# willi-menapace/PlayableEnvironments

Measured on AMD Instinct MI355X. Metric: Mrays/s, higher is better.
Workload: dtype f32; 1 GPU; tennis renderer, 256x256 frame per GPU (rank r renders the frame of seed 1234 + r), 4 objects, 64+128 hierarchical samples/ray (coarse+fine networks), eval - BASELINE.json configs[1]; rays_per_gpu=65536, frames_per_gpu=1, parallelism=frame shard x1

## Files before the change

### playableenvironments_amd/csrc/geometry.hip

```cpp
#include "pr_common.h"

namespace pr {

__global__ void k_camera_rays(int frames, int rays, int per_frame, float half_h, float half_w, const float* __restrict__ c2w,
                              const float* __restrict__ focals, const int32_t* __restrict__ rows,
                              const int32_t* __restrict__ cols, float* __restrict__ origins,
                              float* __restrict__ dirs, float* __restrict__ normals) {
    const long g = (long)blockIdx.x * blockDim.x + threadIdx.x;
    const long total = (long)frames * rays;
    if (g >= total) return;
    const int n = (int)(g / rays);
    const int r = (int)(g - (long)n * rays);
    const float* m = c2w + (size_t)n * 12;
    const float f = focals[n];
    const long pix = per_frame ? g : (long)r;
    const float dx = __fdiv_rn(__fsub_rn((float)cols[pix], half_w), f);
    const float dy = -__fdiv_rn(__fsub_rn((float)rows[pix], half_h), f);
    const float dz = -1.0f;
#pragma unroll
    for (int i = 0; i < 3; ++i) {
        const float v = __fadd_rn(__fadd_rn(__fmul_rn(dx, m[i * 4 + 0]), __fmul_rn(dy, m[i * 4 + 1])),
                                  __fmul_rn(dz, m[i * 4 + 2]));
        dirs[g * 3 + i] = v;
    }
// ... 185 lines not shown
__global__ __launch_bounds__(256) void k_scan_blocks_group(ScanGroup g) {
    scan_blocks_body(g.sums[blockIdx.x], g.offsets[blockIdx.x], g.total[blockIdx.x], g.n);
}

int launch_scan(const int32_t* sums, int32_t* offsets, int32_t* total, int n, hipStream_t s) {
    hipLaunchKernelGGL(k_scan_blocks, dim3(1), dim3(256), 0, s, sums, offsets, total, n);
    PR_LAUNCH_CHECK();
    return PR_OK;
}

__device__ __forceinline__ void fill_body(const FillParams& p) {
    __shared__ int lds[4];
    if (p.skip && *p.skip) return;
    const int lane = threadIdx.x & 63;
    const long g = (long)blockIdx.x * 256 + threadIdx.x;
    const long total = (long)p.frames * p.rays;
    const int P = p.positions;
    ObjRay ray = {};
    bool valid = false;
    int frame = 0;
    if (g < total) {
        const int n = frame = (int)(g / p.rays);
        const float* m = p.w2o + ((size_t)n * p.objects + p.object_index) * 12;
        ray = object_ray(m, p.ray_origins + (size_t)n * 3, p.ray_directions + (size_t)g * 3);
        valid = p.in_scene[(size_t)n * p.objects + p.object_index] != 0;
    }
    const long wave_first = g - lane;
    const RayLanes L(P, lane);
    auto walk = [&](auto&& per_ray) {
        for (int r0 = 0; r0 < 64 && wave_first + r0 < total; r0 += L.per_pass) {
            const int r = r0 + L.sub;
            per_ray(r0, r, wave_first + r < total, broadcast_ray(ray, valid, frame, r), (size_t)(wave_first + r) * P);
        }
    };
    auto inside_at = [&](bool live, const WaveRay& w, size_t base, int i, float* x, float* y, float* z) {
        if (!live || i >= P) return false;
        const float t = p.t[base + i];
        *x = __fadd_rn(w.o[0], __fmul_rn(w.d[0], t));
        *y = __fadd_rn(w.o[1], __fmul_rn(w.d[1], t));
        *z = __fadd_rn(w.o[2], __fmul_rn(w.d[2], t));
        return sample_kept(*x, *y, *z, p.lo, p.hi, p.occ, w.frame);
    };
    int count = 0;
    walk([&](int r0, int r, bool live, const WaveRay& w, size_t base) {
        int ray_count = 0;
        for (int i0 = 0; i0 < P; i0 += L.P2) {
            float x, y, z;
            ray_count += __popcll(L.mine(__ballot(inside_at(live, w, base, i0 + L.idx, &x, &y, &z))));
        }
        L.collect(ray_count, r0, lane, &count);
    });
    int block_total;
    const int first_slot = p.block_offsets[blockIdx.x] + block_exclusive_scan_256(count, lds, &block_total);
    walk([&](int r0, int r, bool live, const WaveRay& w, size_t base) {
        int slot = __shfl(first_slot, r, 64);
        for (int i0 = 0; i0 < P; i0 += L.P2) {
            const int i = i0 + L.idx;
            float x = 0.f, y = 0.f, z = 0.f;
            const bool inside = inside_at(live, w, base, i, &x, &y, &z);
            const unsigned long long mask = L.mine(__ballot(inside));
            if (inside) {
                const int mine = slot + __popcll(mask & ((1ull << L.idx) - 1ull));
                p.rec_pos[(size_t)mine * 3 + 0] = x;
                p.rec_pos[(size_t)mine * 3 + 1] = y;
                p.rec_pos[(size_t)mine * 3 + 2] = z;
                p.rec_flat[mine] = (int32_t)(base + i);
                p.slot[base + i] = mine;
            } else if (live && i < P) {
                p.slot[base + i] = -1;
            }
            slot += __popcll(mask);
        }
    });
}

__global__ __launch_bounds__(256) void k_fill(FillParams p) { fill_body(p); }
struct FillGroup { FillParams p[PR_MAX_OBJECTS]; };
__global__ __launch_bounds__(256) void k_fill_group(FillGroup g) { fill_body(g.p[blockIdx.y]); }

int launch_placement_group(const PlaceParams* pp, const FillParams* fp, int32_t* const* totals, int count, hipStream_t s) {
    if (count <= 0) return PR_OK;
    PR_REQUIRE(count <= PR_MAX_OBJECTS, "placement group: %d objects", count);
    static thread_local PlaceGroup pg;
    static thread_local FillGroup fg;
    ScanGroup sg;
    const long total = (long)pp[0].frames * pp[0].rays;
    const int blocks = (int)((total + 255) / 256);
    for (int k = 0; k < count; ++k) {
        pg.p[k] = pp[k];
        fg.p[k] = fp[k];
        sg.sums[k] = pp[k].block_sums;
        sg.offsets[k] = const_cast<int32_t*>(fp[k].block_offsets);
        sg.total[k] = totals[k];
    }
    sg.n = blocks;
    hipLaunchKernelGGL(k_place_coarse_group, dim3(blocks, count), dim3(256), 0, s, pg);
    PR_LAUNCH_CHECK();
    hipLaunchKernelGGL(k_scan_blocks_group, dim3(count), dim3(256), 0, s, sg);
    PR_LAUNCH_CHECK();
    hipLaunchKernelGGL(k_fill_group, dim3(blocks, count), dim3(256), 0, s, fg);
    PR_LAUNCH_CHECK();
    return PR_OK;
}

int launch_fill(const FillParams& p, hipStream_t s) {
    const long total = (long)p.frames * p.rays;
    const int blocks = (int)((total + 255) / 256);
    hipLaunchKernelGGL(k_fill, dim3(blocks), dim3(256), 0, s, p);
    PR_LAUNCH_CHECK();
    return PR_OK;
}

__device__ __forceinline__ void bitonic_sort_f32(float* key, int n , int lane) {
    for (int k = 2; k <= n; k <<= 1) {
        for (int j = k >> 1; j > 0; j >>= 1) {
            for (int i = lane; i < n; i += 64) {
                const int x = i ^ j;
                if (x > i) {
                    const float a = key[i], b = key[x];
                    const bool up = ((i & k) == 0);
                    if ((a > b) == up) {
                        key[i] = b;
                        key[x] = a;
                    }
                }
            }
            __syncthreads();
        }
    }
}

__global__ __launch_bounds__(64) void k_resample(ResampleParams p, int sort_size) {
    extern __shared__ float sm[];
    if (p.skip && *p.skip) return;
    const int Pc = p.pc, Pf = p.pf;
    float* tc = sm;
    float* al = tc + Pc;
    float* mids = al + Pc;
    float* cdf = mids + Pc;
    float* key = cdf + Pc;
    const int lane = threadIdx.x;
    const long g = blockIdx.x;
    const int n = (int)(g / p.rays);
    const float* m = p.w2o + ((size_t)n * p.objects + p.object_index) * 12;
    const ObjRay ray = object_ray(m, p.ray_origins + (size_t)n * 3, p.ray_directions + (size_t)g * 3);
    const bool valid = p.in_scene[(size_t)n * p.objects + p.object_index] != 0;
    const float norm = sqrtf(__fadd_rn(__fadd_rn(__fmul_rn(ray.d[0], ray.d[0]), __fmul_rn(ray.d[1], ray.d[1])),
                                       __fmul_rn(ray.d[2], ray.d[2])));
    const size_t cbase = (size_t)g * Pc;
    for (int i = lane; i < Pc; i += 64) tc[i] = p.t_coarse[cbase + i];
    __syncthreads();
    for (int i = lane; i < Pc; i += 64) {
        float raw = valid ? p.sigma_coarse[cbase + i] : p.empty_alpha;
        if (noise_present(p.alpha_noise)) raw = __fadd_rn(raw, noise_normal(p.alpha_noise, g, Pc, i));
        const float dt = (i < Pc - 1) ? __fsub_rn(tc[i + 1], tc[i]) : 1e10f;
        const float dist = __fmul_rn(dt, norm);
        const float relu = raw > 0.f ? raw : 0.f;
        al[i] = __fsub_rn(1.0f, expf(__fmul_rn(-relu, dist)));
        if (i < Pc - 1) mids[i] = __fdiv_rn(__fadd_rn(tc[i + 1], tc[i]), 2.0f);
    }
    __syncthreads();
    if (lane == 0) {
        float trans = 1.0f;
        for (int i = 0; i < Pc; ++i) {
            const float a = al[i];
            al[i] = __fmul_rn(a, trans);
            trans = __fmul_rn(trans, __fadd_rn(__fsub_rn(1.0f, a), 1e-10f));
        }
        const int nb = Pc - 2;
        float sum = 0.f;
        for (int j = 0; j < nb; ++j) sum = __fadd_rn(sum, __fadd_rn(al[j + 1], 1e-5f));
        float c = 0.f;
        cdf[0] = 0.f;
        for (int j = 0; j < nb; ++j) {
            c = __fadd_rn(c, __fdiv_rn(__fadd_rn(al[j + 1], 1e-5f), sum));
            cdf[j + 1] = c;
        }
    }
    __syncthreads();
    const int ncdf = Pc - 1;
    for (int i = lane; i < sort_size; i += 64) key[i] = (i < Pc) ? tc[i] : __builtin_inff();
    for (int f = lane; f < Pf; f += 64) {
        const float u = noise_present(p.u_random) ? noise_uniform(p.u_random, g, Pf, f) : p.u_fixed[f];
        int lo_i = 0, hi_i = ncdf;
        while (lo_i < hi_i) {
            const int mid = (lo_i + hi_i) >> 1;
            if (cdf[mid] > u) hi_i = mid; else lo_i = mid + 1;
        }
        const int below = lo_i - 1 < 0 ? 0 : lo_i - 1;
        const int above = lo_i > ncdf - 1 ? ncdf - 1 : lo_i;
        float den = __fsub_rn(cdf[above], cdf[below]);
        if (den < 1e-5f) den = 1.0f;
        const float frac = __fdiv_rn(__fsub_rn(u, cdf[below]), den);
        key[Pc + f] = __fadd_rn(mids[below], __fmul_rn(frac, __fsub_rn(mids[above], mids[below])));
    }
    __syncthreads();
    const int Pm = Pc + Pf;
    float* merged = key + sort_size;
    bool sorted = true;
    for (int i = lane; i + 1 < Pc; i += 64) sorted = sorted && (key[i] <= key[i + 1]);
    for (int f = lane; f + 1 < Pf; f += 64) sorted = sorted && (key[Pc + f] <= key[Pc + f + 1]);
    if (__ballot(sorted) == ~0ull) {
        for (int i = lane; i < Pc; i += 64) {
            const float t = key[i];
            int lo = 0, hi = Pf;
            while (lo < hi) {
                const int mid = (lo + hi) >> 1;
                if (key[Pc + mid] < t) lo = mid + 1; else hi = mid;
            }
            merged[i + lo] = t;
        }
        for (int f = lane; f < Pf; f += 64) {
            const float t = key[Pc + f];
            int lo = 0, hi = Pc;
            while (lo < hi) {
                const int mid = (lo + hi) >> 1;
                if (key[mid] <= t) lo = mid + 1; else hi = mid;
            }
            merged[f + lo] = t;
        }
        __syncthreads();
    } else {
        bitonic_sort_f32(key, sort_size, lane);
        merged = key;
    }
    const size_t fbase = (size_t)g * Pm;
    int count = 0;
    for (int i = lane; i < Pm; i += 64) {
        const float t = merged[i];
        p.t_fine[fbase + i] = t;
        p.sigma_fine[fbase + i] = p.empty_alpha;
        if (p.dispmag_fine) p.dispmag_fine[fbase + i] = 0.f;
        const float x = __fadd_rn(ray.o[0], __fmul_rn(ray.d[0], t));
        const float y = __fadd_rn(ray.o[1], __fmul_rn(ray.d[1], t));
        const float z = __fadd_rn(ray.o[2], __fmul_rn(ray.d[2], t));
        if (sample_kept(x, y, z, p.lo, p.hi, p.occ, n)) ++count;
    }
#pragma unroll
    for (int d = 32; d > 0; d >>= 1) count += __shfl_down(count, d, 64);
    if (lane == 0 && count) atomicAdd(&p.block_sums[g >> 8], count);
}

__global__ __launch_bounds__(256) void k_expected_positions(int frames, int rays, int objects, int object_index, int P,
                                                            const float* ray_origins, const float* ray_directions,
                                                            const float* w2o, const float* t, const float* weights,
                                                            const float* delta, float* expected) {
    const long g = (long)blockIdx.x * 256 + threadIdx.x;
    if (g >= (long)frames * rays) return;
    const int n = (int)(g / rays);
    const ObjRay ray = object_ray(w2o + ((size_t)n * objects + object_index) * 12, ray_origins + (size_t)n * 3,
                                  ray_directions + (size_t)g * 3);
    const size_t base = (size_t)g * P;
    float acc[3] = {0.f, 0.f, 0.f}, wsum = 0.f;
    for (int i = 0; i < P; ++i) {
        const float ti = t[base + i], w = weights[base + i];
        for (int a = 0; a < 3; ++a) {
            float x = __fadd_rn(ray.o[a], __fmul_rn(ray.d[a], ti));
            if (delta) x = __fadd_rn(x, delta[(base + i) * 3 + a]);
            acc[a] = __fadd_rn(acc[a], __fmul_rn(x, w));
        }
        wsum = __fadd_rn(wsum, w);
    }
    for (int a = 0; a < 3; ++a) expected[(size_t)g * 3 + a] = __fdiv_rn(acc[a], __fadd_rn(wsum, 1e-8f));
}

static int next_pow2(int v) {
    int r = 1;
    while (r < v) r <<= 1;
    return r;
}

int launch_resample(const ResampleParams& p, hipStream_t s) {
    PR_REQUIRE(p.pc >= 3, "hierarchical sampling needs at least 3 coarse positions (got %d)", p.pc);
    const long total = (long)p.frames * p.rays;
    const int nblocks256 = (int)((total + 255) / 256);
    PR_TRY(launch_zero_fill(p.block_sums, sizeof(int32_t) * nblocks256, s));
    int sort_size = next_pow2(p.pc + p.pf);
    if (sort_size < 64) sort_size = 64;
    const size_t lds = sizeof(float) * (4 * (size_t)p.pc + 2 * (size_t)sort_size);
    PR_REQUIRE(lds <= 64 * 1024, "resample: too many positions per ray (%d + %d)", p.pc, p.pf);
    hipLaunchKernelGGL(k_resample, dim3((unsigned)total), dim3(64), lds, s, p, sort_size);
    PR_LAUNCH_CHECK();
    return PR_OK;
}

}

extern "C" int pr_expected_positions(int32_t frames, int32_t rays, int32_t objects, int32_t object_index, int32_t positions,
                                     const float* ray_origins, const float* ray_directions, const float* w2o, const float* t,
                                     const float* weights, const float* delta, float* expected, void* stream) {
    PR_REQUIRE(frames > 0 && rays > 0 && positions > 0 && objects > 0 && object_index >= 0 && object_index < objects,
               "pr_expected_positions: bad sizes");
    PR_REQUIRE(ray_origins && ray_directions && w2o && t && weights && expected, "pr_expected_positions: NULL pointer");
    const long total = (long)frames * rays;
    hipLaunchKernelGGL(pr::k_expected_positions, dim3((unsigned)((total + 255) / 256)), dim3(256), 0, (hipStream_t)stream, frames,
                       rays, objects, object_index, positions, ray_origins, ray_directions, w2o, t, weights, delta, expected);
    PR_LAUNCH_CHECK();
    return PR_OK;
}

namespace pr {
struct PatchPixelsParams {
    int frames, objects, height, width, patch, nstrides;
    int strides[4];
    const float* boxes;
    const float* weights;
    const float* u;
    int32_t* rows; int32_t* cols;
    int rays;
};

__global__ __launch_bounds__(256) void k_patch_pixels(PatchPixelsParams p) {
    __shared__ int start[2];
    const int n = blockIdx.x;
    const int H = p.height, W = p.width, K = p.objects;
    const int s0 = p.strides[0], sm = p.strides[p.nstrides - 1];
    if (threadIdx.x < 64) {
        const int lane = threadIdx.x;
        float left[PR_MAX_OBJECTS], right[PR_MAX_OBJECTS], top[PR_MAX_OBJECTS], bottom[PR_MAX_OBJECTS], per[PR_MAX_OBJECTS];
        for (int k = 0; k < K; ++k) {
            const float* b = p.boxes + (size_t)n * 4 * K + k;
            left[k] = fminf(fmaxf(floorf(b[0] * W), 0.f), (float)W);
            top[k] = fminf(fmaxf(floorf(b[K] * H), 0.f), (float)H);
            right[k] = fminf(fmaxf(ceilf(b[2 * K] * W), 0.f), (float)W);
            bottom[k] = fminf(fmaxf(ceilf(b[3 * K] * H), 0.f), (float)H);
            per[k] = p.weights[k] / ((right[k] - left[k]) * (bottom[k] - top[k]));
        }
        auto prefix = [&](long i) -> double {
            const int r = (int)(i / W), c = (int)(i - (long)r * W);
            double acc = 0.0;
            for (int k = 0; k < K; ++k) {
                const double w = right[k] - left[k];
                const double full = fmin((double)r, (double)bottom[k]) - top[k];
                double count = full > 0.0 ? full * w : 0.0;
                if (r >= top[k] && r < bottom[k]) {
                    const double part = fmin((double)(c + 1), (double)right[k]) - left[k];
                    if (part > 0.0) count += part;
                }
                if (count > 0.0) acc += (double)per[k] * count;
            }
            return acc;
        };
        const long total_px = (long)H * W;
        const double total = prefix(total_px - 1);
        long idx = total_px - 1;
        if (total > 0.0 && total < 1e300) {
            const double target = (double)p.u[n] * total;
            long lo = 0, hi = total_px - 1;
            while (lo < hi) {
                const long step = (hi - lo + 64) / 64;
                long cand = lo + (long)(lane + 1) * step - 1;
                if (cand > hi) cand = hi;
                const unsigned long long reached = __ballot(prefix(cand) >= target);
                const int first = reached ? __ffsll((long long)reached) - 1 : 63;
                long part_hi = lo + (long)(first + 1) * step - 1;
                if (part_hi > hi) part_hi = hi;
                lo = lo + (long)first * step;
                hi = part_hi;
            }
            idx = lo;
        }
        const int half = ((p.patch * s0) / sm) / 2;
        int row = (int)(idx / W), col = (int)(idx - (long)row * W);
        row = min(max(row, half * sm), H - sm * (half - 1) - 1);
// ... 407 lines not shown
```

### playableenvironments_amd/csrc/pr_common.h

```cpp
#pragma once

#include <hip/hip_runtime.h>
#include <stdint.h>
#include <stdio.h>
#include <string.h>

#include "playrender.h"

namespace pr {

void set_error(const char* fmt, ...);

#define PR_CHECK_HIP(expr)                                                              \
    do {                                                                                \
        hipError_t _e = (expr);                                                         \
        if (_e != hipSuccess) {                                                         \
            pr::set_error("%s failed: %s (%s:%d)", #expr, hipGetErrorString(_e), __FILE__, __LINE__); \
            return PR_ERR_HIP;                                                          \
        }                                                                               \
    } while (0)

#define PR_REQUIRE(cond, ...)                                                           \
    do {                                                                                \
        if (!(cond)) {                                                                  \
// ... 191 lines not shown
    const float* ptr;
    unsigned int key0, key1;
    int generate;
    int rays, ray_offset, total_rays;
    const unsigned long long* seed_dev;
    unsigned long long salt;
};

__host__ __device__ static inline unsigned long long noise_mix(unsigned long long x) {
    x += 0x9E3779B97F4A7C15ull;
    x = (x ^ (x >> 30)) * 0xBF58476D1CE4E5B9ull;
    x = (x ^ (x >> 27)) * 0x94D049BB133111EBull;
    return x ^ (x >> 31);
}

static inline NoiseRef make_noise(const float* ptr, const pr_call_t& c, int kind, int type, int object) {
    NoiseRef n;
    memset(&n, 0, sizeof(n));
    n.ptr = ptr;
    n.rays = c.rays;
    n.ray_offset = c.noise_ray_offset;
    n.total_rays = c.noise_total_rays > 0 ? c.noise_total_rays : c.rays;
    if (!ptr && (c.flags & PR_FLAG_DEVICE_NOISE)) {
        n.salt = noise_mix((unsigned long long)(kind * 16 + type * 8 + object) + 1);
        const unsigned long long k = noise_mix(c.noise_seed ^ n.salt);
        n.key0 = (unsigned int)k;
        n.key1 = (unsigned int)(k >> 32);
        n.seed_dev = reinterpret_cast<const unsigned long long*>(c.noise_seed_device);
        n.generate = 1;
    }
    return n;
}

static inline NoiseRef perturb_noise(const float* ptr, const pr_call_t& c, int kind, int type, int object) {
    NoiseRef n = make_noise(ptr, c, kind, type, object);
    if (!(c.flags & PR_FLAG_PERTURB)) n.generate = 0;
    return n;
}

struct OccGrid {
    const uint32_t* bits;
    int n[3];
    int words;
    float scale[3];
};
int make_occ_grid(const pr_occupancy_grid_t* g, const pr_object_model_t& m, int object, const char* level, OccGrid* out);

struct PlaceParams {
    int frames, rays, positions, objects, object_index;
    const float* ray_origins;
    const float* ray_directions;
    const float* w2o;
    const uint8_t* in_scene;
    float lo[3], hi[3];
    float z_near_min, z_far_max, empty_alpha;
    const float* linspace;
    NoiseRef jitter;
    float* t;
    float* sigma;
    float* dispmag;
    int32_t* block_sums;
    OccGrid occ;
    const int32_t* skip;
};
int launch_place_coarse(const PlaceParams& p, hipStream_t s);

struct FillParams {
    int frames, rays, positions, objects, object_index;
    const float* ray_origins;
    const float* ray_directions;
    const float* w2o;
    const uint8_t* in_scene;
    float lo[3], hi[3];
    const float* t;
    const int32_t* block_offsets;
    float* rec_pos;
    int32_t* rec_flat;
    int32_t* slot;
    OccGrid occ;
    const int32_t* skip;
};
int launch_fill(const FillParams& p, hipStream_t s);
int launch_placement_group(const PlaceParams* pp, const FillParams* fp, int32_t* const* totals, int count, hipStream_t s);

int launch_scan(const int32_t* sums, int32_t* offsets, int32_t* total, int n, hipStream_t s);

struct ResampleParams {
    int frames, rays, objects, object_index;
    int pc, pf;
    const float* ray_origins;
    const float* ray_directions;
    const float* w2o;
    const uint8_t* in_scene;
    float lo[3], hi[3];
    float empty_alpha;
    const float* t_coarse;
    const float* sigma_coarse;
    NoiseRef alpha_noise;
    const float* u_fixed;
    NoiseRef u_random;
    float* t_fine;
    float* sigma_fine;
    float* dispmag_fine;
    int32_t* block_sums;
    OccGrid occ;
    const int32_t* skip;
};
int launch_resample(const ResampleParams& p, hipStream_t s);

struct FoldParams {
    int frames, objects, object_index;
    const float* style;
    int S;
    pr_linear_t affine1; const float* bn1_mean; const float* bn1_var;
    pr_linear_t affine4; const float* bn4_mean; const float* bn4_var;
    float eps;
    int W, Wpad, W2, W2pad;
    float* table;
    int row_floats;
};
int launch_adain_fold(const FoldParams& p, hipStream_t s);
int launch_adain_fold_group(const FoldParams* jobs, int count, hipStream_t s);

int launch_mlp(const MlpParams& p, int max_rows, bool naive, const pr_object_model_t* raw, hipStream_t s);
int launch_mlp_group(const MlpParams* host_jobs, const int* max_rows, int count, hipStream_t s);
int launch_mlp_split(const MlpParams& p, int max_rows, int terms, hipStream_t s);
int launch_mlp_split_group(const MlpParams* host_jobs, const int* max_rows, int count, int terms, hipStream_t s);
int launch_mlp_sigma(const MlpParams& p, int max_rows, hipStream_t s);
int launch_mlp_split_sigma(const MlpParams& p, int max_rows, int terms, hipStream_t s);

struct BnFinalizeParams {
    const double* stats;
    const int32_t* count;
    int width, width_pad;
    float momentum;
    float* running_mean;
    float* running_var;
    long long* num_batches_tracked;
    float* batch_mean;
    float* batch_var;
    int frozen;
};
int launch_bn_finalize(const BnFinalizeParams& p, hipStream_t s);

struct BnFoldJob {
    const double* stats; const int32_t* count; int width, width_pad; float momentum;
    float* running_mean; float* running_var; long long* num_batches_tracked;
    float* batch_mean; float* batch_var; int frozen;
    const float* style; int style_stride, S, frames;
    pr_linear_t affine; float eps;
    float* table; int row_floats, g_off, b_off;
    int32_t* normalised_out;
};
struct BnFoldJobs { BnFoldJob job[PR_MAX_OBJECTS]; };
int launch_bn_fold_group(const BnFoldJobs& jobs, int count, hipStream_t s);

struct DivChainJob {
    const int32_t* total; const int32_t* rec_flat; const int32_t* row_flags; const float* rec_pos;
    NoiseRef noise; int positions;
    const float* bin; int bin_pad, benc, b_octaves;
    const unsigned char* bbits; size_t bbits_stride;
    int BW, BWpad, b_count, b_skip;
    Seg seg0[PR_MAX_LAYERS]; Seg seg1;
    const float* w_out;
    const float* braw;
    float lo[3], hi[3];
    int canonical;
    float* div;
    int32_t* tile_counter;
};
bool div_chain_supported(int BWpad, int bin_pad);
int launch_div_chain_group(const DivChainJob* jobs, const long* max_rows, int count, hipStream_t s);

struct CompositeObject {
    const float* t;
    const float* sigma;
    const int32_t* slot;
    const float* divergence;
    const float* dispmag;
    const float* feat;
    NoiseRef noise;
    int positions;
    pr_entry_t out;
};
struct CompositeParams {
    int frames, rays, objects, static_objects, F;
    int fix_overlaps;
    int any_divergence;
    int sigmoid;
    int total_positions;
    int sort_size;
// ... 326 lines not shown
```

### playableenvironments_amd/csrc/render.hip

```cpp
#include "pr_common.h"

#include <stdarg.h>

#include <atomic>
#include <mutex>
#include <vector>

namespace pr {

struct ProfileRecord { int category; hipEvent_t start, stop; };
static std::atomic<bool> g_profile_on{false};
static std::vector<ProfileRecord> g_profile;
static std::mutex g_profile_mutex;

int prepare_kernel(const void* kernel, int lds_bytes, int* cu_count) {
    struct Entry { const void* kernel; int device; int cus; };
    static std::vector<Entry> done;
    static std::mutex guard;
    int dev = 0;
    PR_CHECK_HIP(hipGetDevice(&dev));
    std::lock_guard<std::mutex> lock(guard);
    for (const Entry& e : done)
        if (e.kernel == kernel && e.device == dev) {
            if (cu_count) *cu_count = e.cus;
// ... 207 lines not shown
    }
    if (gate_active(c)) {
        plan->pend_act = take(sizeof(float) * (size_t)MAX_RESIDENT_TILES * TILE_M * MAX_WIDTH);
        plan->pend_meta = take(sizeof(int32_t) * (size_t)MAX_RESIDENT_TILES * TILE_M * 2);
    }
    if (defer_active(c, objs)) {
        ModelDims d0;
        PR_TRY(compute_dims(objs[0].coarse, &d0));
        plan->pooled = take(sizeof(float) * 2 * (size_t)c.objects * nr * hidden_row_floats(d0.W2));
    }
    if (c.flags & (PR_FLAG_TRAIN_BN | PR_FLAG_SAVE_FOR_BACKWARD)) {
        plan->h1 = take(sizeof(float) * max_cap * MAX_WIDTH);
        plan->h2 = take(sizeof(float) * max_cap * (MAX_WIDTH / 2 + 32));
        plan->row_flags = take(sizeof(int32_t) * max_cap);
        plan->batch_stats = take(sizeof(float) * 4 * MAX_WIDTH);
    }
    if (div_t) {
        plan->div_t0 = take(sizeof(float) * div_t0);
        plan->div_ta = take(sizeof(float) * div_t);
        plan->div_tb = take(sizeof(float) * div_t);
    }
    if (c.flags & PR_FLAG_SAVE_FOR_BACKWARD) {
        for (int t = 0; t < ntypes; ++t) {
            const size_t arena = take(feat_bytes[t]);
            for (int k = 0; k < c.objects; ++k) plan->type[t].feat[k] += arena;
        }
    } else {
        const size_t arena = take(feat_bytes[0] > feat_bytes[1] ? feat_bytes[0] : feat_bytes[1]);
        for (int t = 0; t < ntypes; ++t)
            for (int k = 0; k < c.objects; ++k) plan->type[t].feat[k] += arena;
    }
    plan->bytes = off;
    return PR_OK;
}

bool group_active(const pr_call_t& c) {
    return !(c.flags & (PR_FLAG_TRAIN_BN | PR_FLAG_SAVE_FOR_BACKWARD | PR_FLAG_NAIVE_MLP)) && c.objects > 1;
}

bool group_train_active(const pr_call_t& c) {
    return (c.flags & PR_FLAG_SAVE_FOR_BACKWARD) && !(c.flags & PR_FLAG_NAIVE_MLP) && c.objects > 1;
}

void bbox_split(const pr_object_model_t& m, float* lo, float* hi, float* size) {
    for (int a = 0; a < 3; ++a) {
        lo[a] = m.bbox[2 * a];
        hi[a] = m.bbox[2 * a + 1];
        if (size) size[a] = m.bbox[2 * a + 1] - m.bbox[2 * a];
    }
}

struct SampleArrays { float* t; float* sigma; int32_t* slot; float* dispmag; float* feat; };
static SampleArrays sample_arrays(const Plan& plan, char* ws, const RetainCtx* rc, int t, int k, bool has_bender) {
    SampleArrays a;
    if (rc && ((rc->mask >> k) & 1u)) {
        const RetainObjectPlan& o = rc->plan.obj[k];
        a.t = reinterpret_cast<float*>(rc->base + o.t[t]);
        a.sigma = reinterpret_cast<float*>(rc->base + o.sigma[t]);
        a.slot = reinterpret_cast<int32_t*>(rc->base + o.slot[t]);
        a.dispmag = has_bender ? reinterpret_cast<float*>(rc->base + o.dispmag[t]) : nullptr;
        a.feat = reinterpret_cast<float*>(rc->base + o.feat[t]);
        return a;
    }
    const TypePlan& tp = plan.type[t];
    a.t = reinterpret_cast<float*>(ws + tp.t[k]);
    a.sigma = reinterpret_cast<float*>(ws + tp.sigma[k]);
    a.slot = reinterpret_cast<int32_t*>(ws + tp.slot[k]);
    a.dispmag = has_bender ? reinterpret_cast<float*>(ws + tp.dispmag[k]) : nullptr;
    a.feat = reinterpret_cast<float*>(ws + tp.feat[k]);
    return a;
}

static int render(const pr_call_t& c, const pr_object_t* objs, const pr_occupancy_t* occupancy, const RetainCtx* rc,
                  const pr_outputs_t* outs[2], char* ws, const Plan& plan, hipStream_t s) {
    const int ntypes = c.use_fine ? 2 : 1;
    const int K = c.objects;
    if (rc) PR_TRY(launch_retain_probe(c, objs, *rc, s));
    int32_t* block_sums_all = reinterpret_cast<int32_t*>(ws + plan.block_sums);
    int32_t* block_offsets_all = reinterpret_cast<int32_t*>(ws + plan.block_offsets);
    const bool place_grouped = c.objects > 1 && ((c.flags & PR_FLAG_SAVE_FOR_BACKWARD) || group_active(c));
    static thread_local PlaceParams place_jobs[PR_MAX_OBJECTS];
    static thread_local FillParams fill_jobs[PR_MAX_OBJECTS];
    int32_t* total_ptrs[PR_MAX_OBJECTS];
    float* rec_pos = reinterpret_cast<float*>(ws + plan.rec_pos);
    int32_t* rec_flat = reinterpret_cast<int32_t*>(ws + plan.rec_flat);
    const bool naive = (c.flags & PR_FLAG_NAIVE_MLP) != 0;
    const bool gate = gate_active(c);
    const bool defer = defer_active(c, objs);
    const bool grouped = group_active(c);
    MlpParams jobs[PR_MAX_OBJECTS];
    int job_rows[PR_MAX_OBJECTS];
    FoldParams fold_jobs[PR_MAX_OBJECTS];
    const bool train_grouped = group_train_active(c);
    struct TrainJob {
        MlpParams mp; FoldParams fo; ModelDims d; const pr_object_model_t* m; const SavedPlan* sv;
        double* stats; int32_t* stat_count; float* batch; float* h1; float* h2; float* rec_pos; int32_t* rec_flat;
        int k, P, max_tiles; bool frozen, save;
    };
    static thread_local TrainJob train_jobs[PR_MAX_OBJECTS];

    for (int t = 0; t < ntypes; ++t) {
        const TypePlan& tp = plan.type[t];
        int32_t* totals = reinterpret_cast<int32_t*>(ws + tp.totals);
        int32_t* head_counts = reinterpret_cast<int32_t*>(ws + tp.head_counts);
        PR_TRY(launch_zero_fill(ws + tp.zero_begin, tp.zero_bytes, s));
        const pr_noise_t& noise = t ? c.noise_fine : c.noise_coarse;
        int total_positions = 0;
        auto finish_object = [&](TrainJob& J, int stage, bool launch) -> int {
            MlpParams& mp = J.mp; FoldParams& fo = J.fo; const ModelDims& d = J.d; const pr_object_model_t& m = *J.m;
            const SavedPlan& sv = *J.sv;
            double* stats = J.stats; int32_t* stat_count = J.stat_count; float* batch = J.batch; float* h1 = J.h1; float* h2 = J.h2;
            float* rec_pos = J.rec_pos; int32_t* rec_flat = J.rec_flat;
            const int k = J.k, P = J.P, max_tiles = J.max_tiles;
            const bool frozen = J.frozen, save = J.save;
            BnFinalizeParams bf;
            memset(&bf, 0, sizeof(bf));
            bf.count = stat_count; bf.momentum = 0.1f;
            bf.frozen = frozen ? 1 : 0;
            if (stage == 1) {
                bf.stats = stats; bf.width = d.W; bf.width_pad = d.Wpad;
                bf.running_mean = m.bn1_mean; bf.running_var = m.bn1_var; bf.num_batches_tracked = (long long*)m.bn1_batches;
                bf.batch_mean = batch; bf.batch_var = batch + MAX_WIDTH;
                PR_TRY(launch_bn_finalize(bf, s));
                fo.bn1_mean = batch; fo.bn1_var = batch + MAX_WIDTH;
                PR_TRY(launch_adain_fold(fo, s));
                mp.phase = 2; mp.h_in = h1; mp.h_in_width = d.Wpad; mp.h_out = h2; mp.h_out_width = d.W2pad;
                mp.stats = stats + 2 * MAX_WIDTH;
                if (launch) PR_TRY(launch_mlp(mp, max_tiles, false, &m, s));
                return PR_OK;
            }
            if (stage == 2) {
                bf.stats = stats + 2 * MAX_WIDTH; bf.width = d.W2; bf.width_pad = d.W2pad;
                bf.running_mean = m.bn4_mean; bf.running_var = m.bn4_var; bf.num_batches_tracked = (long long*)m.bn4_batches;
                bf.batch_mean = batch + 2 * MAX_WIDTH; bf.batch_var = batch + 3 * MAX_WIDTH;
                PR_TRY(launch_bn_finalize(bf, s));
                fo.bn4_mean = batch + 2 * MAX_WIDTH; fo.bn4_var = batch + 3 * MAX_WIDTH;
                PR_TRY(launch_adain_fold(fo, s));
                mp.phase = 3; mp.h_in = h2; mp.h_in_width = d.W2pad; mp.h_out = nullptr;
                if (launch) PR_TRY(launch_mlp(mp, max_tiles, false, &m, s));
                return PR_OK;
            }
            if (outs[t] && outs[t]->normalised_samples)
                PR_CHECK_HIP(hipMemcpyAsync(outs[t]->normalised_samples + k, stat_count, sizeof(int32_t),
                                            hipMemcpyDeviceToDevice, s));
            if (save && m.has_bender) {
                const size_t cap_rows = (size_t)c.frames * c.rays * P;
                float* div = reinterpret_cast<float*>(ws + sv.div);
                NoiseRef probes = make_noise(noise.divergence[k], c, NOISE_DIVERGENCE, t, k);
                if (!(c.flags & PR_FLAG_TRAIN_BN)) probes.generate = 0;
                if (probes.ptr || probes.generate) {
                    DivergenceParams dp;
                    memset(&dp, 0, sizeof(dp));
                    dp.total = totals + k; dp.max_rows = (int)cap_rows;
                    dp.rec_flat = rec_flat; dp.row_flags = mp.row_flags; dp.rec_pos = rec_pos;
                    dp.noise = probes; dp.positions = P;
                    dp.bin = mp.save_bin; dp.bin_pad = d.bin_pad; dp.benc = d.benc; dp.b_octaves = m.bender_octaves;
                    dp.bacts = mp.save_bact; dp.bact_stride = mp.save_bact_stride; dp.BW = d.BW; dp.BWpad = d.BWpad;
                    dp.b_count = m.bender_count; dp.b_skip = m.bender_skip; dp.bin_real = d.bin;
                    dp.layers = m.bender; dp.out_head = m.bender_out; dp.braw = mp.save_braw;
                    bbox_split(m, dp.lo, dp.hi, nullptr);
                    dp.canonical = (c.flags & PR_FLAG_CANONICAL_POSE) ? 1 : 0;
                    dp.t0 = reinterpret_cast<float*>(ws + plan.div_t0);
                    dp.ta = reinterpret_cast<float*>(ws + plan.div_ta);
                    dp.tb = reinterpret_cast<float*>(ws + plan.div_tb);
                    dp.div = div;
                    PR_TRY(launch_divergence(dp, s));
                }
            }
            return PR_OK;
        };
        for (int pass = (place_grouped && t == 0) ? 0 : 1; pass < 2; ++pass) {
        if (pass == 1 && place_grouped && t == 0) PR_TRY(launch_placement_group(place_jobs, fill_jobs, total_ptrs, K, s));
        for (int k = 0; k < K; ++k) {
            const pr_object_model_t& m = t ? objs[k].fine : objs[k].coarse;
            const float* packed = static_cast<const float*>(t ? objs[k].packed_fine : objs[k].packed_coarse);
            ModelDims d;
            PackedLayout l;
            PR_TRY(compute_dims(m, &d));
            PR_TRY(compute_layout(m, d, &l));
            const int P = m.positions;
            if (pass == 1) total_positions += P;
            int32_t* block_sums = block_sums_all + (size_t)k * plan.nblocks256;
            int32_t* block_offsets = block_offsets_all + (size_t)k * plan.nblocks256;
            const bool placed = place_grouped && t == 0;
            const SampleArrays arr = sample_arrays(plan, ws, rc, t, k, m.has_bender != 0);
            float* t_arr = arr.t;
            float* sigma = arr.sigma;
            int32_t* slot = arr.slot;
            float* dispmag = arr.dispmag;
            float* feat = arr.feat;
            const int32_t* skip = (rc && ((rc->mask >> k) & 1u)) ? &rc->hdr->reuse[k] : nullptr;
            float* adain = reinterpret_cast<float*>(ws + tp.adain[k]);
            const bool save = (c.flags & PR_FLAG_SAVE_FOR_BACKWARD) != 0;
            const SavedPlan& sv = tp.saved[k];
            OccGrid occ;
            PR_TRY(make_occ_grid(occupancy ? (t ? &occupancy->fine[k] : &occupancy->coarse[k]) : nullptr, m, k, t ? "fine" : "coarse", &occ));
            if (save) {
                rec_pos = reinterpret_cast<float*>(ws + sv.rec_pos);
                rec_flat = reinterpret_cast<int32_t*>(ws + sv.rec_flat);
            } else if (grouped) {
                rec_pos = reinterpret_cast<float*>(ws + plan.rec_pos_k[k]);
                rec_flat = reinterpret_cast<int32_t*>(ws + plan.rec_flat_k[k]);
            }

            if (t == 0) {
                PlaceParams pp;
                memset(&pp, 0, sizeof(pp));
                pp.frames = c.frames; pp.rays = c.rays; pp.positions = P; pp.objects = K; pp.object_index = k;
                pp.ray_origins = c.ray_origins; pp.ray_directions = c.ray_directions; pp.w2o = c.w2o;
                pp.in_scene = c.object_in_scene;
                bbox_split(m, pp.lo, pp.hi, nullptr);
                pp.z_near_min = m.z_near_min; pp.z_far_max = m.z_far_max; pp.empty_alpha = m.empty_space_alpha;
                pp.linspace = c.linspace_coarse[k];
                pp.jitter = perturb_noise(c.noise_coarse.jitter[k], c, NOISE_JITTER, 0, k);
                pp.t = t_arr; pp.sigma = sigma; pp.dispmag = dispmag; pp.block_sums = block_sums;
                pp.occ = occ;
                pp.skip = skip;
                if (pass == 0) place_jobs[k] = pp;
                else if (!placed) PR_TRY(launch_place_coarse(pp, s));
            } else {
                ResampleParams rp;
                memset(&rp, 0, sizeof(rp));
                rp.frames = c.frames; rp.rays = c.rays; rp.objects = K; rp.object_index = k;
                rp.pc = objs[k].coarse.positions; rp.pf = c.positions_fine[k];
                rp.ray_origins = c.ray_origins; rp.ray_directions = c.ray_directions; rp.w2o = c.w2o;
                rp.in_scene = c.object_in_scene;
                bbox_split(m, rp.lo, rp.hi, nullptr);
                rp.empty_alpha = m.empty_space_alpha;
                const SampleArrays coarse_arr = sample_arrays(plan, ws, rc, 0, k, objs[k].coarse.has_bender != 0);
                rp.t_coarse = coarse_arr.t;
                rp.sigma_coarse = coarse_arr.sigma;
                rp.alpha_noise = perturb_noise(c.noise_coarse.alpha[k], c, NOISE_ALPHA, 0, k);
                rp.u_fixed = c.linspace_fine[k];
                rp.u_random = perturb_noise(c.noise_coarse.pdf[k], c, NOISE_PDF, 0, k);
                rp.t_fine = t_arr; rp.sigma_fine = sigma; rp.dispmag_fine = dispmag; rp.block_sums = block_sums;
                rp.occ = occ;
                rp.skip = skip;
                PR_TRY(launch_resample(rp, s));
            }
            if (pass == 1 && !placed) PR_TRY(launch_scan(block_sums, block_offsets, totals + k, plan.nblocks256, s));

            FillParams fp;
            memset(&fp, 0, sizeof(fp));
            fp.frames = c.frames; fp.rays = c.rays; fp.positions = P; fp.objects = K; fp.object_index = k;
            fp.ray_origins = c.ray_origins; fp.ray_directions = c.ray_directions; fp.w2o = c.w2o;
            fp.in_scene = c.object_in_scene;
            bbox_split(m, fp.lo, fp.hi, nullptr);
            fp.t = t_arr; fp.block_offsets = block_offsets; fp.rec_pos = rec_pos; fp.rec_flat = rec_flat; fp.slot = slot;
            fp.occ = occ;
            fp.skip = skip;
            if (pass == 0) {
                fill_jobs[k] = fp;
                total_ptrs[k] = totals + k;
                continue;
            }
            if (!placed) PR_TRY(launch_fill(fp, s));

            FoldParams fo;
            memset(&fo, 0, sizeof(fo));
            fo.frames = c.frames; fo.objects = K; fo.object_index = k;
            fo.style = c.style; fo.S = m.style_features;
            fo.affine1 = m.affine1; fo.bn1_mean = m.bn1_mean; fo.bn1_var = m.bn1_var;
            fo.affine4 = m.affine4; fo.bn4_mean = m.bn4_mean; fo.bn4_var = m.bn4_var;
            fo.eps = m.bn_eps;
            fo.W = d.W; fo.Wpad = d.Wpad; fo.W2 = d.W2; fo.W2pad = d.W2pad;
            fo.table = adain; fo.row_floats = adain_row_floats(d);

            MlpParams mp;
            memset(&mp, 0, sizeof(mp));
            const bool split3 = train_grouped && (c.flags & PR_FLAG_SPLIT_BACKWARD) && (c.flags & PR_FLAG_SAVE_FOR_BACKWARD);
            PR_TRY(build_mlp_layers(m, d, l, packed, &mp, split3));
            mp.rec_pos = rec_pos; mp.rec_flat = rec_flat; mp.total = totals + k;
            mp.samples_per_frame = c.rays * P; mp.positions = P; mp.rays = c.rays;
            mp.canonical = (c.flags & PR_FLAG_CANONICAL_POSE) ? 1 : 0;
            bbox_split(m, mp.lo, mp.hi, mp.size);
            mp.empty_alpha = m.empty_space_alpha;
            mp.in_scene = c.object_in_scene + k; mp.in_scene_stride = K;
            mp.ray_directions = c.ray_directions; mp.ray_origins = c.ray_origins;
            mp.w2o = c.w2o + (size_t)k * 12; mp.w2o_stride = K * 12;
            mp.deformation = c.deformation + (size_t)k * m.deformation_features;
            mp.deformation_stride = K * m.deformation_features;
            mp.adain = adain; mp.adain_stride = fo.row_floats;
            mp.sigma = sigma; mp.dispmag = dispmag; mp.feat = feat;
            if (defer) {
                mp.n_layers = mp.n_backbone + 2;
                mp.F = hidden_row_floats(d.W2);
                mp.ones_col = d.W2;
            }
            if (gate) {
                mp.gate = 1;
                mp.pend_act = reinterpret_cast<float*>(ws + plan.pend_act);
                mp.pend_meta = reinterpret_cast<int32_t*>(ws + plan.pend_meta);
                mp.head_count = head_counts + k;
            }
            mp.tile_counter = head_counts + PR_MAX_OBJECTS + k;
            if (outs[t] && outs[t]->sample_delta[k]) {
                PR_TRY(launch_zero_fill(outs[t]->sample_delta[k], sizeof(float) * 3 * (size_t)c.frames * c.rays * P, s));
                if (m.has_bender) mp.delta_dense = outs[t]->sample_delta[k];
            }
            const size_t cap = (size_t)c.frames * c.rays * P;
            const int max_tiles = (int)cap;
            if (!(c.flags & (PR_FLAG_TRAIN_BN | PR_FLAG_SAVE_FOR_BACKWARD))) {
                if (grouped) {
                    fold_jobs[k] = fo;
                    jobs[k] = mp;
                    job_rows[k] = max_tiles;
                    continue;
                }
                if (rc) PR_TRY(launch_retain_gate(*rc, totals, k, 1, s));
                PR_TRY(launch_adain_fold(fo, s));
                if (c.precision != PR_PRECISION_FP32 && !naive)
                    PR_TRY(launch_mlp_split(mp, max_tiles, c.precision == PR_PRECISION_F16 ? 1 : 3, s));
                else
                    PR_TRY(launch_mlp(mp, max_tiles, naive, &m, s));
            } else {
                const bool frozen = !(c.flags & PR_FLAG_TRAIN_BN);
                PR_REQUIRE(!naive, "the scalar debugging kernel has no train-mode BatchNorm");
                double* stats = reinterpret_cast<double*>(ws + sv.stats);
                int32_t* stat_count = reinterpret_cast<int32_t*>(ws + sv.stat_count);
                float* batch = reinterpret_cast<float*>(ws + (save ? sv.batch : plan.batch_stats));
                float* h1 = reinterpret_cast<float*>(ws + (save ? sv.h1 : plan.h1));
                float* h2 = reinterpret_cast<float*>(ws + (save ? sv.h2 : plan.h2));
                mp.row_flags = reinterpret_cast<int32_t*>(ws + (save ? sv.row_flags : plan.row_flags));
                mp.stat_count = stat_count;
                if (save) {
                    const size_t cap_rows = (size_t)c.frames * c.rays * P;
                    mp.save_enc = reinterpret_cast<float*>(ws + sv.enc);
                    mp.save_act = reinterpret_cast<float*>(ws + sv.act);
                    mp.save_act_stride = cap_rows * d.Wpad;
                    mp.save_bits = reinterpret_cast<unsigned char*>(ws + sv.bits);
                    mp.save_bits_stride = relu_bits_bytes(cap_rows, d.Wpad);
                    if (m.has_bender) {
                        mp.save_bin = reinterpret_cast<float*>(ws + sv.bin);
                        mp.save_bact = reinterpret_cast<float*>(ws + sv.bact);
                        mp.save_bact_stride = cap_rows * d.BWpad;
                        mp.save_bbits = reinterpret_cast<unsigned char*>(ws + sv.bbits);
// ... 323 lines not shown
```

Baseline: 0.3302 Mrays/s.

## Batch fine-level resampling across objects into one grouped multi-wave kernel

Adds a grouped resample kernel that processes all objects in a single launch. Each 256-thread block handles 64 rays, with the sequential transmittance and CDF chain computed one ray per lane. Per-wave LDS barriers replace workgroup barriers in the bitonic sort, and the fine-level scan and fill are grouped the same way as the coarse placement path. This cuts launch count and the heavily serialized one-wave-per-ray structure, at the cost of more LDS per block and a serial per-lane CDF loop.

```diff
diff --git a/playableenvironments_amd/csrc/geometry.hip b/playableenvironments_amd/csrc/geometry.hip
--- a/playableenvironments_amd/csrc/geometry.hip
+++ b/playableenvironments_amd/csrc/geometry.hip
@@ -291,20 +291,32 @@
     if (count <= 0) return PR_OK;
     PR_REQUIRE(count <= PR_MAX_OBJECTS, "placement group: %d objects", count);
     static thread_local PlaceGroup pg;
-    static thread_local FillGroup fg;
-    ScanGroup sg;
+    const int32_t* sums[PR_MAX_OBJECTS];
     const long total = (long)pp[0].frames * pp[0].rays;
     const int blocks = (int)((total + 255) / 256);
     for (int k = 0; k < count; ++k) {
         pg.p[k] = pp[k];
+        sums[k] = pp[k].block_sums;
+    }
+    hipLaunchKernelGGL(k_place_coarse_group, dim3(blocks, count), dim3(256), 0, s, pg);
+    PR_LAUNCH_CHECK();
+    return launch_compaction_group(fp, sums, totals, count, s);
+}
+
+int launch_compaction_group(const FillParams* fp, const int32_t* const* sums, int32_t* const* totals, int count, hipStream_t s) {
+    if (count <= 0) return PR_OK;
+    PR_REQUIRE(count <= PR_MAX_OBJECTS, "compaction group: %d objects", count);
+    static thread_local FillGroup fg;
+    ScanGroup sg;
+    const long total = (long)fp[0].frames * fp[0].rays;
+    const int blocks = (int)((total + 255) / 256);
+    for (int k = 0; k < count; ++k) {
         fg.p[k] = fp[k];
-        sg.sums[k] = pp[k].block_sums;
+        sg.sums[k] = sums[k];
         sg.offsets[k] = const_cast<int32_t*>(fp[k].block_offsets);
         sg.total[k] = totals[k];
     }
     sg.n = blocks;
-    hipLaunchKernelGGL(k_place_coarse_group, dim3(blocks, count), dim3(256), 0, s, pg);
-    PR_LAUNCH_CHECK();
     hipLaunchKernelGGL(k_scan_blocks_group, dim3(count), dim3(256), 0, s, sg);
     PR_LAUNCH_CHECK();
     hipLaunchKernelGGL(k_fill_group, dim3(blocks, count), dim3(256), 0, s, fg);
@@ -320,6 +332,13 @@
     return PR_OK;
 }
 
+__device__ __forceinline__ void wave_sync_lds() {
+    __builtin_amdgcn_fence(__ATOMIC_RELEASE, "workgroup");
+    __builtin_amdgcn_wave_barrier();
+    __builtin_amdgcn_fence(__ATOMIC_ACQUIRE, "workgroup");
+}
+
+template <bool kWave = false>
 __device__ __forceinline__ void bitonic_sort_f32(float* key, int n , int lane) {
     for (int k = 2; k <= n; k <<= 1) {
         for (int j = k >> 1; j > 0; j >>= 1) {
@@ -334,7 +353,7 @@
                     }
                 }
             }
-            __syncthreads();
+            if (kWave) wave_sync_lds(); else __syncthreads();
         }
     }
 }
@@ -450,6 +469,155 @@
     if (lane == 0 && count) atomicAdd(&p.block_sums[g >> 8], count);
 }
 
+constexpr int RG_PAIRS = 64;
+constexpr int RG_WAVES = 4;
+struct ResampleGroup { ResampleParams p[PR_MAX_OBJECTS]; int sort_size[PR_MAX_OBJECTS]; };
+
+static size_t resample_group_lds(int pc, int sort_size) {
+    return sizeof(float) * ((size_t)RG_PAIRS * (pc | 1) + (size_t)RG_WAVES * (2 * (size_t)pc + 2 * (size_t)sort_size));
+}
+
+__global__ __launch_bounds__(64 * RG_WAVES) void k_resample_group(ResampleGroup grp) {
+    extern __shared__ float sm[];
+    const ResampleParams p = grp.p[blockIdx.y];
+    if (p.skip && *p.skip) return;
+    const int sort_size = grp.sort_size[blockIdx.y];
+    const int Pc = p.pc, Pf = p.pf;
+    const int stride = Pc | 1;
+    const int lane = threadIdx.x & 63, wave = threadIdx.x >> 6;
+    float* chain = sm;
+    float* tc = sm + RG_PAIRS * stride + wave * (2 * Pc + 2 * sort_size);
+    float* mids = tc + Pc;
+    float* key = mids + Pc;
+    float* merged_buf = key + sort_size;
+    const long total = (long)p.frames * p.rays;
+    const long g0 = (long)blockIdx.x * RG_PAIRS;
+    constexpr int PER_WAVE = RG_PAIRS / RG_WAVES;
+
+    for (int q = 0; q < PER_WAVE; ++q) {
+        const int pair = wave * PER_WAVE + q;
+        const long g = g0 + pair;
+        if (g >= total) break;
+        const int n = (int)(g / p.rays);
+        const float* m = p.w2o + ((size_t)n * p.objects + p.object_index) * 12;
+        const ObjRay ray = object_ray(m, p.ray_origins + (size_t)n * 3, p.ray_directions + (size_t)g * 3);
+        const bool valid = p.in_scene[(size_t)n * p.objects + p.object_index] != 0;
+        const float norm = sqrtf(__fadd_rn(__fadd_rn(__fmul_rn(ray.d[0], ray.d[0]), __fmul_rn(ray.d[1], ray.d[1])),
+                                           __fmul_rn(ray.d[2], ray.d[2])));
+        const size_t cbase = (size_t)g * Pc;
+        float* al = chain + pair * stride;
+        for (int i = lane; i < Pc; i += 64) tc[i] = p.t_coarse[cbase + i];
+        wave_sync_lds();
+        for (int i = lane; i < Pc; i += 64) {
+            float raw = valid ? p.sigma_coarse[cbase + i] : p.empty_alpha;
+            if (noise_present(p.alpha_noise)) raw = __fadd_rn(raw, noise_normal(p.alpha_noise, g, Pc, i));
+            const float dt = (i < Pc - 1) ? __fsub_rn(tc[i + 1], tc[i]) : 1e10f;
+            const float dist = __fmul_rn(dt, norm);
+            const float relu = raw > 0.f ? raw : 0.f;
+            al[i] = __fsub_rn(1.0f, expf(__fmul_rn(-relu, dist)));
+        }
+        wave_sync_lds();
+    }
+    __syncthreads();
+
+    if (wave == 0 && g0 + lane < total) {
+        float* al = chain + lane * stride;
+        float trans = 1.0f;
+        for (int i = 0; i < Pc; ++i) {
+            const float a = al[i];
+            al[i] = __fmul_rn(a, trans);
+            trans = __fmul_rn(trans, __fadd_rn(__fsub_rn(1.0f, a), 1e-10f));
+        }
+        const int nb = Pc - 2;
+        float sum = 0.f;
+        for (int j = 0; j < nb; ++j) sum = __fadd_rn(sum, __fadd_rn(al[j + 1], 1e-5f));
+        float c = 0.f;
+        al[0] = 0.f;
+        for (int j = 0; j < nb; ++j) {
+            c = __fadd_rn(c, __fdiv_rn(__fadd_rn(al[j + 1], 1e-5f), sum));
+            al[j + 1] = c;
+        }
+    }
+    __syncthreads();
+
+    const int ncdf = Pc - 1;
+    const int Pm = Pc + Pf;
+    int count = 0;
+    for (int q = 0; q < PER_WAVE; ++q) {
+        const int pair = wave * PER_WAVE + q;
+        const long g = g0 + pair;
+        if (g >= total) break;
+        const int n = (int)(g / p.rays);
+        const float* m = p.w2o + ((size_t)n * p.objects + p.object_index) * 12;
+        const ObjRay ray = object_ray(m, p.ray_origins + (size_t)n * 3, p.ray_directions + (size_t)g * 3);
+        const size_t cbase = (size_t)g * Pc;
+        const float* cdf = chain + pair * stride;
+        for (int i = lane; i < Pc; i += 64) tc[i] = p.t_coarse[cbase + i];
+        wave_sync_lds();
+        for (int i = lane; i + 1 < Pc; i += 64) mids[i] = __fdiv_rn(__fadd_rn(tc[i + 1], tc[i]), 2.0f);
+        for (int i = lane; i < sort_size; i += 64) key[i] = (i < Pc) ? tc[i] : __builtin_inff();
+        wave_sync_lds();
+        for (int f = lane; f < Pf; f += 64) {
+            const float u = noise_present(p.u_random) ? noise_uniform(p.u_random, g, Pf, f) : p.u_fixed[f];
+            int lo_i = 0, hi_i = ncdf;
+            while (lo_i < hi_i) {
+                const int mid = (lo_i + hi_i) >> 1;
+                if (cdf[mid] > u) hi_i = mid; else lo_i = mid + 1;
+            }
+            const int below = lo_i - 1 < 0 ? 0 : lo_i - 1;
+            const int above = lo_i > ncdf - 1 ? ncdf - 1 : lo_i;
+            float den = __fsub_rn(cdf[above], cdf[below]);
+            if (den < 1e-5f) den = 1.0f;
+            const float frac = __fdiv_rn(__fsub_rn(u, cdf[below]), den);
+            key[Pc + f] = __fadd_rn(mids[below], __fmul_rn(frac, __fsub_rn(mids[above], mids[below])));
+        }
+        wave_sync_lds();
+        float* merged = merged_buf;
+        bool sorted = true;
+        for (int i = lane; i + 1 < Pc; i += 64) sorted = sorted && (key[i] <= key[i + 1]);
+        for (int f = lane; f + 1 < Pf; f += 64) sorted = sorted && (key[Pc + f] <= key[Pc + f + 1]);
+        if (__ballot(sorted) == ~0ull) {
+            for (int i = lane; i < Pc; i += 64) {
+                const float t = key[i];
+                int lo = 0, hi = Pf;
+                while (lo < hi) {
+                    const int mid = (lo + hi) >> 1;
+                    if (key[Pc + mid] < t) lo = mid + 1; else hi = mid;
+                }
+                merged[i + lo] = t;
+            }
+            for (int f = lane; f < Pf; f += 64) {
+                const float t = key[Pc + f];
+                int lo = 0, hi = Pc;
+                while (lo < hi) {
+                    const int mid = (lo + hi) >> 1;
+                    if (key[mid] <= t) lo = mid + 1; else hi = mid;
+                }
+                merged[f + lo] = t;
+            }
+            wave_sync_lds();
+        } else {
+            bitonic_sort_f32<true>(key, sort_size, lane);
+            merged = key;
+        }
+        const size_t fbase = (size_t)g * Pm;
+        for (int i = lane; i < Pm; i += 64) {
+            const float t = merged[i];
+            p.t_fine[fbase + i] = t;
+            p.sigma_fine[fbase + i] = p.empty_alpha;
+            if (p.dispmag_fine) p.dispmag_fine[fbase + i] = 0.f;
+            const float x = __fadd_rn(ray.o[0], __fmul_rn(ray.d[0], t));
+            const float y = __fadd_rn(ray.o[1], __fmul_rn(ray.d[1], t));
+            const float z = __fadd_rn(ray.o[2], __fmul_rn(ray.d[2], t));
+            if (sample_kept(x, y, z, p.lo, p.hi, p.occ, n)) ++count;
+        }
+        wave_sync_lds();
+    }
+#pragma unroll
+    for (int d = 32; d > 0; d >>= 1) count += __shfl_down(count, d, 64);
+    if (lane == 0 && count) atomicAdd(&p.block_sums[(g0 + wave * PER_WAVE) >> 8], count);
+}
+
 __global__ __launch_bounds__(256) void k_expected_positions(int frames, int rays, int objects, int object_index, int P,
                                                             const float* ray_origins, const float* ray_directions,
                                                             const float* w2o, const float* t, const float* weights,
@@ -489,6 +657,34 @@
     const size_t lds = sizeof(float) * (4 * (size_t)p.pc + 2 * (size_t)sort_size);
     PR_REQUIRE(lds <= 64 * 1024, "resample: too many positions per ray (%d + %d)", p.pc, p.pf);
     hipLaunchKernelGGL(k_resample, dim3((unsigned)total), dim3(64), lds, s, p, sort_size);
+    PR_LAUNCH_CHECK();
+    return PR_OK;
+}
+
+int launch_resample_group(const ResampleParams* rp, int count, hipStream_t s) {
+    if (count <= 0) return PR_OK;
+    PR_REQUIRE(count <= PR_MAX_OBJECTS, "resample group: %d objects", count);
+    static thread_local ResampleGroup rg;
+    const long total = (long)rp[0].frames * rp[0].rays;
+    const int nblocks256 = (int)((total + 255) / 256);
+    size_t lds = 0;
+    for (int k = 0; k < count; ++k) {
+        PR_REQUIRE(rp[k].pc >= 3, "hierarchical sampling needs at least 3 coarse positions (got %d)", rp[k].pc);
+        PR_REQUIRE(rp[k].block_sums == rp[0].block_sums + (size_t)k * nblocks256, "resample group: block sums must be contiguous");
+        int sort_size = next_pow2(rp[k].pc + rp[k].pf);
+        if (sort_size < 64) sort_size = 64;
+        rg.p[k] = rp[k];
+        rg.sort_size[k] = sort_size;
+        const size_t need = resample_group_lds(rp[k].pc, sort_size);
+        if (need > lds) lds = need;
+    }
+    if (lds > 64 * 1024) {
+        for (int k = 0; k < count; ++k) PR_TRY(launch_resample(rp[k], s));
+        return PR_OK;
+    }
+    PR_TRY(launch_zero_fill(rp[0].block_sums, sizeof(int32_t) * (size_t)count * nblocks256, s));
+    const unsigned blocks = (unsigned)((total + RG_PAIRS - 1) / RG_PAIRS);
+    hipLaunchKernelGGL(k_resample_group, dim3(blocks, count), dim3(64 * RG_WAVES), lds, s, rg);
     PR_LAUNCH_CHECK();
     return PR_OK;
 }
diff --git a/playableenvironments_amd/csrc/pr_common.h b/playableenvironments_amd/csrc/pr_common.h
--- a/playableenvironments_amd/csrc/pr_common.h
+++ b/playableenvironments_amd/csrc/pr_common.h
@@ -297,6 +297,7 @@
 };
 int launch_fill(const FillParams& p, hipStream_t s);
 int launch_placement_group(const PlaceParams* pp, const FillParams* fp, int32_t* const* totals, int count, hipStream_t s);
+int launch_compaction_group(const FillParams* fp, const int32_t* const* sums, int32_t* const* totals, int count, hipStream_t s);
 
 int launch_scan(const int32_t* sums, int32_t* offsets, int32_t* total, int n, hipStream_t s);
 
@@ -322,6 +323,7 @@
     const int32_t* skip;
 };
 int launch_resample(const ResampleParams& p, hipStream_t s);
+int launch_resample_group(const ResampleParams* rp, int count, hipStream_t s);
 
 struct FoldParams {
     int frames, objects, object_index;
diff --git a/playableenvironments_amd/csrc/render.hip b/playableenvironments_amd/csrc/render.hip
--- a/playableenvironments_amd/csrc/render.hip
+++ b/playableenvironments_amd/csrc/render.hip
@@ -313,6 +313,9 @@
     static thread_local PlaceParams place_jobs[PR_MAX_OBJECTS];
     static thread_local FillParams fill_jobs[PR_MAX_OBJECTS];
     int32_t* total_ptrs[PR_MAX_OBJECTS];
+    const bool fine_grouped = c.objects > 1 && group_active(c) && !(c.flags & (PR_FLAG_SAVE_FOR_BACKWARD | PR_FLAG_TRAIN_BN));
+    static thread_local ResampleParams resample_jobs[PR_MAX_OBJECTS];
+    const int32_t* sum_ptrs[PR_MAX_OBJECTS];
     float* rec_pos = reinterpret_cast<float*>(ws + plan.rec_pos);
     int32_t* rec_flat = reinterpret_cast<int32_t*>(ws + plan.rec_flat);
     const bool naive = (c.flags & PR_FLAG_NAIVE_MLP) != 0;
@@ -400,8 +403,16 @@
             }
             return PR_OK;
         };
-        for (int pass = (place_grouped && t == 0) ? 0 : 1; pass < 2; ++pass) {
-        if (pass == 1 && place_grouped && t == 0) PR_TRY(launch_placement_group(place_jobs, fill_jobs, total_ptrs, K, s));
+        const bool level_grouped = t == 0 ? place_grouped : fine_grouped;
+        for (int pass = level_grouped ? 0 : 1; pass < 2; ++pass) {
+        if (pass == 1 && level_grouped) {
+            if (t == 0) {
+                PR_TRY(launch_placement_group(place_jobs, fill_jobs, total_ptrs, K, s));
+            } else {
+                PR_TRY(launch_resample_group(resample_jobs, K, s));
+                PR_TRY(launch_compaction_group(fill_jobs, sum_ptrs, total_ptrs, K, s));
+            }
+        }
         for (int k = 0; k < K; ++k) {
             const pr_object_model_t& m = t ? objs[k].fine : objs[k].coarse;
             const float* packed = static_cast<const float*>(t ? objs[k].packed_fine : objs[k].packed_coarse);
@@ -413,7 +424,7 @@
             if (pass == 1) total_positions += P;
             int32_t* block_sums = block_sums_all + (size_t)k * plan.nblocks256;
             int32_t* block_offsets = block_offsets_all + (size_t)k * plan.nblocks256;
-            const bool placed = place_grouped && t == 0;
+            const bool placed = level_grouped;
             const SampleArrays arr = sample_arrays(plan, ws, rc, t, k, m.has_bender != 0);
             float* t_arr = arr.t;
             float* sigma = arr.sigma;
@@ -467,7 +478,8 @@
                 rp.t_fine = t_arr; rp.sigma_fine = sigma; rp.dispmag_fine = dispmag; rp.block_sums = block_sums;
                 rp.occ = occ;
                 rp.skip = skip;
-                PR_TRY(launch_resample(rp, s));
+                if (pass == 0) resample_jobs[k] = rp;
+                else if (!placed) PR_TRY(launch_resample(rp, s));
             }
             if (pass == 1 && !placed) PR_TRY(launch_scan(block_sums, block_offsets, totals + k, plan.nblocks256, s));
 
@@ -483,6 +495,7 @@
             if (pass == 0) {
                 fill_jobs[k] = fp;
                 total_ptrs[k] = totals + k;
+                sum_ptrs[k] = block_sums;
                 continue;
             }
             if (!placed) PR_TRY(launch_fill(fp, s));
```

Result: no change. 0.3317 Mrays/s, median of 6 (+0.5%).
